# proroklab/DVM-SLAM

Measured on AMD Instinct MI355X. Metric: frames/sec ORB extract+match 640x480x8lvl, higher is better.
Workload: dtype u8; 1 GPU; single agent tracking front end: 640x480 8-level ORB extract (1000 features) + frame-to-frame windowed Hamming match, one agent per GPU; frames_per_launch_group=256, resident_stream_frames=1024, nfeatures=1000, nlevels=8, ini_th_fast=20, min_th_fast=7, match=SearchByProjection(Cur,Last) window th=15, parallelism=agents1, pipeline_lanes=2, stream_texture=rich

## Files before the change

dvm_slam_amd/capi.py:

```python
from __future__ import annotations

import ctypes as C
import os

import numpy as np

_HERE = os.path.dirname(os.path.abspath(__file__))
LIB_PATH = os.environ.get("DVM_HIP_LIB") or os.path.join(_HERE, "lib", "libdvmslam_hip.so")

DVM_OK = 0
ERRORS = {-1: "DVM_ERR_INVALID", -2: "DVM_ERR_EMPTY", -3: "DVM_ERR_CAPACITY", -4: "DVM_ERR_HIP",
          -5: "DVM_ERR_NO_DEVICE", -6: "DVM_ERR_STATE"}

KP_DTYPE = np.dtype([("x", "<f4"), ("y", "<f4"), ("size", "<f4"), ("angle", "<f4"), ("response", "<f4"),
                     ("octave", "<i4"), ("class_id", "<i4")])
MATCH_DTYPE = np.dtype([("best_idx", "<i4"), ("best_dist", "<i4"), ("second_dist", "<i4"),
                        ("best_level", "<i2"), ("second_level", "<i2")])


class DvmError(RuntimeError):
    def __init__(self, code, msg):
        super().__init__(f"{ERRORS.get(code, code)}: {msg}")
        self.code = code

# ... 242 lines not shown
        kps = np.zeros(cap, KP_DTYPE)
        desc = np.zeros((cap, 32), np.uint8)
        n, mono = C.c_int(0), C.c_int(0)
        rc = self.L.dvm_orb_download(self.h, frame, _p(kps), _p(desc), cap, C.byref(n), C.byref(mono))
        if rc == -3 and n.value > cap:
            return self.download(frame, cap=n.value)
        check(rc)
        return n.value, kps[:n.value].copy(), desc[:n.value].copy(), mono.value

    def result_device(self, frame=0):
        k, d, n = C.c_void_p(), C.c_void_p(), C.c_void_p()
        cap = C.c_int(0)
        check(self.L.dvm_orb_result_device(self.h, frame, C.byref(k), C.byref(d), C.byref(n), C.byref(cap)))
        return k.value, d.value, n.value, cap.value

    def copy_result(self, frame, d_kps, d_desc, d_n):
        check(self.L.dvm_orb_copy_result(self.h, frame, C.c_void_p(d_kps), C.c_void_p(d_desc), C.c_void_p(d_n)))

    def scale_factors_device(self):
        return self.L.dvm_orb_scale_factors_device(self.h)

    def pyramid(self, frame, level):
        ptr = C.c_void_p()
        r, c, s = C.c_int(0), C.c_int(0), C.c_int(0)
        check(self.L.dvm_orb_pyramid(self.h, frame, level, C.byref(ptr), C.byref(r), C.byref(c), C.byref(s)))
        return ptr.value, r.value, c.value, s.value

    def debug_level(self, frame, level, bordered=False):
        _, r, c, _ = self.pyramid(frame, level)
        out = np.zeros((r + 38, c + 38) if bordered else (r, c), np.uint8)
        check(self.L.dvm_orb_debug_level(self.h, frame, level, int(bordered), _p(out)))
        return out

    def debug_blurred(self, frame, level):
        _, r, c, _ = self.pyramid(frame, level)
        out = np.zeros((r, c), np.uint8)
        check(self.L.dvm_orb_debug_blurred(self.h, frame, level, _p(out)))
        return out

    def debug_candidates(self, frame, level, cap=300000):
        xs, ys, sc = (np.zeros(cap, np.int32) for _ in range(3))
        n = C.c_int(0)
        check(self.L.dvm_orb_debug_candidates(self.h, frame, level, _p(xs), _p(ys), _p(sc), cap, C.byref(n)))
        return xs[:n.value].copy(), ys[:n.value].copy(), sc[:n.value].copy()

    def debug_level_keypoints(self, frame, level, cap=20000):
        k = np.zeros(cap, KP_DTYPE)
        n = C.c_int(0)
        check(self.L.dvm_orb_debug_level_keypoints(self.h, frame, level, _p(k), cap, C.byref(n)))
        return k[:n.value].copy()

    def profiling(self, on=True):
        check(self.L.dvm_orb_profiling(self.h, int(on)))

    def profile_reset(self):
        check(self.L.dvm_orb_profile_reset(self.h))

    def profile_get(self, name):
        ms, cnt = C.c_double(0), C.c_int64(0)
        rc = self.L.dvm_orb_profile_get(self.h, name.encode(), C.byref(ms), C.byref(cnt))
        return (ms.value, cnt.value) if rc == 0 else (0.0, 0)

    def stream(self):
        return self.L.dvm_orb_stream(self.h)


# ... 1993 lines not shown
```

dvm_slam_amd/csrc/capi.cpp:

```cpp
#include <algorithm>
#include <cstring>
#include <new>
#include <string>
#include <type_traits>
#include <mutex>
#include <unordered_map>
#include <vector>

#include "../../include/dvmslam_hip.h"
#include "camera_model.h"
#include "chain.h"
#include "match_kernels.h"
#include "orb_pipeline.h"

namespace dvm {
const char* last_error_cstr();
}
using namespace dvm;

struct dvm_orb {
  OrbPipeline* p;
  float* d_scale = nullptr;
  uint64_t id = 0, serial = 0;
  int last_n = 0;
// ... 142 lines not shown
}
const float* dvm_orb_scale_factors_device(dvm_orb* h) { return h ? h->d_scale : nullptr; }
int dvm_orb_download(dvm_orb* h, int frame, dvm_keypoint* kps, uint8_t* desc, int cap, int* n, int* mono_index) {
  if (!h) return DVM_ERR_INVALID;
  return h->p->download(frame, kps, desc, cap, n, mono_index);
}
int dvm_orb_download_batch(dvm_orb* h, int count, dvm_keypoint* const* kps, uint8_t* const* desc, const int* caps, int* n, int* mono_index) {
  if (!h || !caps) return DVM_ERR_INVALID;
  return h->p->download_batch(count, kps, desc, caps, n, mono_index);
}
int dvm_orb_pyramid(dvm_orb* h, int frame, int level, const uint8_t** d_ptr, int* rows, int* cols, int* stride) {
  if (!h || !h->p->configured) return DVM_ERR_STATE;
  OrbPipeline& P = *h->p;
  if (level < 0 || level >= P.PD.nlevels || frame < 0 || frame >= P.max_batch) return DVM_ERR_INVALID;
  const LevelDesc& L = P.PD.lv[level];
  if (d_ptr) *d_ptr = P.d_pyr + (size_t)frame * P.PD.pyr_frame_bytes + L.pyr_off + (size_t)kEdge * L.stride + kEdge;
  if (rows) *rows = L.h;
  if (cols) *cols = L.w;
  if (stride) *stride = L.stride;
  return DVM_OK;
}

int dvm_orb_debug_level(dvm_orb* h, int frame, int level, int bordered, uint8_t* out) {
  if (!h || !h->p->configured || !out) return DVM_ERR_STATE;
  OrbPipeline& P = *h->p;
  if (level < 0 || level >= P.PD.nlevels || frame < 0 || frame >= P.last_batch) return DVM_ERR_INVALID;
  int rc = P.sync();
  if (rc != DVM_OK) return rc;
  const LevelDesc& L = P.PD.lv[level];
  const uint8_t* base = P.d_pyr + (size_t)frame * P.PD.pyr_frame_bytes + L.pyr_off;
  if (bordered)
    return hip_check(hipMemcpy2D(out, L.w + 2 * kEdge, base, L.stride, L.w + 2 * kEdge, L.h + 2 * kEdge, hipMemcpyDeviceToHost), "memcpy2d");
  return hip_check(hipMemcpy2D(out, L.w, base + (size_t)kEdge * L.stride + kEdge, L.stride, L.w, L.h, hipMemcpyDeviceToHost), "memcpy2d");
}
int dvm_orb_debug_blurred(dvm_orb* h, int frame, int level, uint8_t* out) {
  if (!h || !h->p->configured || !out) return DVM_ERR_STATE;
  OrbPipeline& P = *h->p;
  if (level < 0 || level >= P.PD.nlevels || frame < 0 || frame >= P.last_batch) return DVM_ERR_INVALID;
  int rc = P.refresh_blur();
  if (rc == DVM_OK) rc = P.sync();
  if (rc != DVM_OK) return rc;
  const LevelDesc& L = P.PD.lv[level];
  return hip_check(hipMemcpy2D(out, L.w, P.d_blur + (size_t)frame * P.PD.blur_frame_bytes + L.blur_off, L.blur_stride, L.w, L.h,
                               hipMemcpyDeviceToHost), "memcpy2d");
}
int dvm_orb_debug_candidates(dvm_orb* h, int frame, int level, int32_t* xs, int32_t* ys, int32_t* scores, int cap, int* n) {
  if (!h || !h->p->configured) return DVM_ERR_STATE;
  OrbPipeline& P = *h->p;
  if (level < 0 || level >= P.PD.nlevels || frame < 0 || frame >= P.last_batch) return DVM_ERR_INVALID;
  int rc = P.sync();
  if (rc != DVM_OK) return rc;
  const LevelDesc& LD = P.PD.lv[level];
  std::vector<int32_t> cc(std::max(LD.cell_count, 1));
  if (LD.cell_count > 0) {
    rc = hip_check(hipMemcpy(cc.data(), P.d_cell_count + (size_t)frame * P.PD.ncells + LD.cell_first, (size_t)LD.cell_count * 4, hipMemcpyDeviceToHost), "memcpy");
    if (rc != DVM_OK) return rc;
  }
  int cnt = 0;
  for (int c = 0; c < LD.cell_count; c++) cnt += cc[c];
  if (n) *n = cnt;
  if (cnt > cap) return DVM_ERR_CAPACITY;
  std::vector<uint32_t> tmp(cnt > 0 ? cnt : 1);
  for (int c = 0, o = 0; c < LD.cell_count; c++) {
    if (cc[c] > 0) {
      rc = hip_check(hipMemcpy(tmp.data() + o, P.d_cand + (size_t)frame * P.PD.cand_frame_slots + P.cells[LD.cell_first + c].cand_base,
                               (size_t)cc[c] * 4, hipMemcpyDeviceToHost), "memcpy");
// ... 986 lines not shown
```

dvm_slam_amd/csrc/orb_kernels.h:

```cpp
#pragma once
#include <hip/hip_runtime.h>
#include <stdint.h>

#include "orb_device.h"

namespace dvm {

struct dvm_keypoint_pod {
  float x, y, size, angle, response;
  int32_t octave, class_id;
};

struct HostMirror {
  dvm_keypoint_pod* kps = nullptr;
  uint8_t* desc = nullptr;
  int32_t* n = nullptr;
  int32_t* mono = nullptr;
};

void upload_constants(const int8_t* disc_u, const int8_t* disc_v, const int* gauss7);
void launch_pyr_level0(hipStream_t s, const uint8_t* d_src, int rows, int cols, int sstride, int64_t frame_stride,
                       uint8_t* d_pyr, const PipelineDesc& PD, int batch);
void launch_pyr_resize(hipStream_t s, uint8_t* d_pyr, const PipelineDesc& PD, int level, const int32_t* d_tabs, int batch);
void launch_pyr_borders(hipStream_t s, uint8_t* d_pyr, const PipelineDesc& PD, int batch);
void launch_fast(hipStream_t s, const uint8_t* d_pyr, const CellDesc* d_cells, const PipelineDesc& PD, uint32_t* d_cand,
                 int32_t* d_cell_count, int batch, int max_rw, int max_rh, int cell_first, int cell_num, const CellDesc* h_cells);
int octree_root_nodes(const LevelDesc& L);
bool raise_dynamic_lds(const void* fn, int bytes);
bool octree_fits_device(const PipelineDesc& PD);
bool octree_prepare_device(const PipelineDesc& PD);
void launch_octree(hipStream_t s, const uint32_t* d_cand, const int32_t* d_cell_count, const CellDesc* d_cells, uint32_t* d_dense,
                   int32_t* d_lvl_count, const PipelineDesc& PD, int32_t* d_nid, uint32_t* d_sel, int32_t* d_nsel, int32_t* d_err,
                   int batch, int level_first, int level_num, bool latency = false);
bool octree_blur_fits(const PipelineDesc& PD);
void launch_octree_blur(hipStream_t s, const uint32_t* d_cand, const int32_t* d_cell_count, const CellDesc* d_cells, uint32_t* d_dense,
                        int32_t* d_lvl_count, const PipelineDesc& PD, int32_t* d_nid, uint32_t* d_sel, int32_t* d_nsel, int32_t* d_err, int batch,
                        const uint8_t* d_pyr, uint8_t* d_blur, const TileDesc* d_tiles, const int* gauss7);
void launch_assemble(hipStream_t s, const uint32_t* d_sel, const int32_t* d_nsel, const PipelineDesc& PD, int lap0,
                     int lap1, dvm_keypoint_pod* d_kps, KpAux* d_aux, int32_t* d_n, int32_t* d_mono, int batch,
                     HostMirror hm = HostMirror());
void launch_blur(hipStream_t s, const uint8_t* d_pyr, uint8_t* d_blur, const TileDesc* d_tiles, const PipelineDesc& PD,
                 const int32_t* d_lvl_start, int batch);
void launch_orient_desc(hipStream_t s, const uint8_t* d_pyr, const uint8_t* d_blur, const PipelineDesc& PD,
                        const KpAux* d_aux, const int32_t* d_n, dvm_keypoint_pod* d_kps, uint8_t* d_desc, int batch,
                        HostMirror hm = HostMirror());
void launch_orient_desc_blur(hipStream_t s, const uint8_t* d_pyr, const PipelineDesc& PD, const KpAux* d_aux, const int32_t* d_n,
                             dvm_keypoint_pod* d_kps, uint8_t* d_desc, int batch, HostMirror hm = HostMirror());
void launch_copy_result(hipStream_t s, const dvm_keypoint_pod* kps_src, dvm_keypoint_pod* kps_dst, const uint8_t* desc_src, uint8_t* desc_dst, int cap,
                        const int32_t* n_src, int32_t* n_dst);

}
```

dvm_slam_amd/csrc/orb_kernels.hip:

```cpp
#include <hip/hip_runtime.h>

#include <map>
#include <mutex>
#include <utility>

#include <algorithm>
#include <cstdlib>

#include "orb_device.h"
#include "orb_kernels.h"
#include "blur_tile.h"

#pragma clang fp contract(off)

namespace dvm {

__constant__ int c_pattern[1024] = {
#include "orb_pattern_31.inc"
};
__constant__ int8_t c_circle[16][2] = {{0, 3},  {1, 3},   {2, 2},   {3, 1},   {3, 0},  {3, -1}, {2, -2}, {1, -3},
                                       {0, -3}, {-1, -3}, {-2, -2}, {-3, -1}, {-3, 0}, {-3, 1}, {-2, 2}, {-1, 3}};
__device__ uint2 c_disc_w[256];
__device__ uint2 c_disc_w43[512];
__constant__ int c_gauss7[7];
// ... 164 lines not shown
  if (X4 >= bw) return;
  uint8_t* Dl = pyr + (int64_t)f * pyr_frame_bytes + L.pyr_off;
#pragma unroll
  for (int rr = 0; rr < TH / 4; rr++) {
    const int dy = y0 + ty + 4 * rr;
    if (dy >= L.h) break;
    const int sy = sy_[rr];
    const int r0 = min(max(sy, 0), P.h - 1) - sya, r1 = min(max(sy + 1, 0), P.h - 1) - sya;
    const uint32_t bb = bb_[rr];
    const uint32_t b0 = bb & 0xFFFFu, b1 = bb >> 16;
    const uint8_t* S0 = rz_smem + r0 * lds_pitch;
    const uint8_t* S1 = rz_smem + r1 * lds_pitch;
    uint32_t v = 0;
#pragma unroll
    for (int k = 0; k < 4; k++) {
      const uint32_t s00 = S0[sx[k]], s01 = S0[sx[k] + 1], s10 = S1[sx[k]], s11 = S1[sx[k] + 1];
      const uint32_t h0 = udot2(s00 | (s01 << 16), al[k], 0u);
      const uint32_t h1 = udot2(s10 | (s11 << 16), al[k], 0u);
      const uint32_t r = ((__umul24(b0, h0 >> 4) >> 16) + (__umul24(b1, h1 >> 4) >> 16) + 2u) >> 2;
      v |= r << (8 * k);
    }
    *reinterpret_cast<uint32_t*>(Dl + (int64_t)(kEdge + dy) * L.stride + X4) = v;
    int top, bot;
    mirror_rows(dy, L.h, top, bot);
    if (top >= 0) *reinterpret_cast<uint32_t*>(Dl + (int64_t)top * L.stride + X4) = v;
    if (bot >= 0) *reinterpret_cast<uint32_t*>(Dl + (int64_t)bot * L.stride + X4) = v;
  }
}

template <int TH>
__global__ void __launch_bounds__(256) k_pyr_resize(uint8_t* __restrict__ pyr, int pyr_frame_bytes, LevelDesc P,
                                                    LevelDesc L, const int32_t* __restrict__ tabs, int lds_pitch) {
  pyr_resize_tile<TH>(pyr, pyr_frame_bytes, P, L, tabs, lds_pitch, blockIdx.z, blockIdx.x, blockIdx.y);
}

__global__ void __launch_bounds__(256) k_pyr_borders(uint8_t* __restrict__ pyr, PipelineDesc PD, int strip_blocks) {
  const int f = blockIdx.z, tid = threadIdx.x;
  if ((int)blockIdx.y < strip_blocks) {
    const int sr = blockIdx.y * 4 + (tid >> 6);
    if (sr >= 2 * kEdge * PD.nlevels) return;
    const LevelDesc& L = PD.lv[sr / (2 * kEdge)];
    const int r = sr % (2 * kEdge);
    const int row = r < kEdge ? r : L.h + r;
    const int X = 32 + (blockIdx.x * 64 + (tid & 63)) * 16;
    if (X + 16 > L.w + kEdge) return;
    uint8_t* base = pyr + (int64_t)f * PD.pyr_frame_bytes + L.pyr_off;
    const uint8_t* S = base + (int64_t)(kEdge + reflect101(row - kEdge, L.h)) * L.stride;
    *reinterpret_cast<uint4*>(base + (int64_t)row * L.stride + X) = *reinterpret_cast<const uint4*>(S + X);
    return;
  }
  if (blockIdx.x != 0) return;
  int g = ((int)blockIdx.y - strip_blocks) * 128 + (tid >> 1), lvl = 0;
  while (lvl < PD.nlevels && g >= PD.lv[lvl].h + 2 * kEdge) { g -= PD.lv[lvl].h + 2 * kEdge; lvl++; }
  if (lvl >= PD.nlevels) return;
  const LevelDesc& L = PD.lv[lvl];
  const int w = L.w;
  const bool strip = g < kEdge || g >= L.h + kEdge;
  uint8_t* base = pyr + (int64_t)f * PD.pyr_frame_bytes + L.pyr_off;
  uint8_t* D = base + (int64_t)g * L.stride;
  const uint8_t* S = base + (int64_t)(kEdge + reflect101(g - kEdge, L.h)) * L.stride;
  uint32_t* D32 = reinterpret_cast<uint32_t*>(D);
  const uint32_t* S32 = reinterpret_cast<const uint32_t*>(S);
  if (w < 40) {
    if (tid & 1) return;
    for (int X = 0; X < w + 2 * kEdge; X++)
      if (strip || X < kEdge || X >= w + kEdge) D[X] = S[kEdge + reflect101(X - kEdge, w)];
// ... 1019 lines not shown
  uint2 w[256];
  for (int i = 0; i < 256; i++) w[i] = make_uint2(0u, 0u);
  for (int p = 0; p < kDiscPixels; p++) {
    const int u = disc_u[p], v = disc_v[p];
    const int item = (v + kHalfPatch) * 8 + ((u + kHalfPatch) >> 2), k = (u + kHalfPatch) & 3;
    w[item].x |= (uint32_t)(u + 16) << (8 * k);
    w[item].y |= 1u << (8 * k);
  }
  hipMemcpyToSymbol(HIP_SYMBOL(c_disc_w), w, sizeof(w));
  uint2 w43[512];
  for (int i = 0; i < 512; i++) w43[i] = make_uint2(0u, 0u);
  for (int p = 0; p < kDiscPixels; p++) {
    const int u = disc_u[p], v = disc_v[p];
    const int item = (v + kPbR) * kPbDw + ((u + kPbR) >> 2), k = (u + kPbR) & 3;
    w43[item].x |= (uint32_t)(u + 16) << (8 * k);
    w43[item].y |= 1u << (8 * k);
  }
  hipMemcpyToSymbol(HIP_SYMBOL(c_disc_w43), w43, sizeof(w43));
  hipMemcpyToSymbol(HIP_SYMBOL(c_gauss7), gauss7, 7 * sizeof(int));
}

void launch_pyr_level0(hipStream_t s, const uint8_t* d_src, int rows, int cols, int sstride, int64_t frame_stride,
                       uint8_t* d_pyr, const PipelineDesc& PD, int batch) {
  const LevelDesc& L = PD.lv[0];
  dim3 grid(cdiv(cdiv(L.w + 2 * kEdge, 16), 64), cdiv(L.h, 16), batch);
  hipLaunchKernelGGL(k_pyr_level0, grid, dim3(256), 0, s, d_src, rows, cols, sstride, frame_stride, d_pyr,
                     PD.pyr_frame_bytes, L);
}
void launch_pyr_resize(hipStream_t s, uint8_t* d_pyr, const PipelineDesc& PD, int level, const int32_t* d_tabs, int batch) {
  const LevelDesc& L = PD.lv[level];
  const LevelDesc& P = PD.lv[level - 1];
  const double sxs = (double)P.w / L.w, sys = (double)P.h / L.h;
  const int pitch = (((int)(kRzTW * sxs) + 16) + 3) & ~3;
  if (batch <= 8) {
    const int nrows = (int)(16 * sys) + 4;
    dim3 grid(cdiv(L.w + 2 * kEdge, kRzTW), cdiv(L.h, 16), batch);
    hipLaunchKernelGGL(k_pyr_resize<16>, grid, dim3(256), (size_t)pitch * nrows, s, d_pyr, PD.pyr_frame_bytes, P, L, d_tabs, pitch);
    return;
  }
  const int nrows = (int)(kRzTH * sys) + 4;
  dim3 grid(cdiv(L.w + 2 * kEdge, kRzTW), cdiv(L.h, kRzTH), batch);
  hipLaunchKernelGGL(k_pyr_resize<kRzTH>, grid, dim3(256), (size_t)pitch * nrows, s, d_pyr, PD.pyr_frame_bytes, P, L, d_tabs, pitch);
}
void launch_pyr_borders(hipStream_t s, uint8_t* d_pyr, const PipelineDesc& PD, int batch) {
  int rows = 0, maxw = 0;
  for (int l = 0; l < PD.nlevels; l++) { rows += PD.lv[l].h + 2 * kEdge; maxw = std::max(maxw, PD.lv[l].w + 2 * kEdge); }
  const int strip_blocks = cdiv(2 * kEdge * PD.nlevels, 4);
  dim3 grid(std::max(1, cdiv(cdiv(maxw, 16), 64)), strip_blocks + cdiv(rows, 128), batch);
  hipLaunchKernelGGL(k_pyr_borders, grid, dim3(256), 0, s, d_pyr, PD, strip_blocks);
}
static void launch_fast_wide(hipStream_t s, const uint8_t* d_pyr, const CellDesc* d_cells, const PipelineDesc& PD, uint32_t* d_cand,
                             int32_t* d_cell_count, int batch, int max_rw, int max_rh, int cell_first, int cell_num) {
  const FastLds lay = fast_lds_layout(max_rw, max_rh);
  const dim3 grid(cell_num * 8 * ((batch + 8 * kFastFramesPerWG - 1) / (8 * kFastFramesPerWG)));
  const bool small = (max_rw - 6) * (max_rh - 6) <= 32 * 128;
  static const int lds_pad = std::getenv("DVM_FAST_LDS_PAD") ? atoi(std::getenv("DVM_FAST_LDS_PAD")) : 0;
#define DVM_FAST_LAUNCH(P, W)                                                                                              \
  do {                                                                                                                     \
    if (lay.total() > 48 * 1024)                                                                                           \
      raise_dynamic_lds(reinterpret_cast<const void*>(k_fast_cells<P, W>), lay.total());                                   \
    hipLaunchKernelGGL((k_fast_cells<P, W>), grid, dim3(64 * W), lay.total() + lds_pad, s, d_pyr, PD.pyr_frame_bytes, d_cells, PD,   \
                       d_cand, d_cell_count, max_rw, max_rh, batch, cell_first, cell_num);                                 \
  } while (0)
  if (lay.tile_pitch == 64) { if (small) DVM_FAST_LAUNCH(64, 2); else DVM_FAST_LAUNCH(64, 4); }
  else DVM_FAST_LAUNCH(0, 4);
#undef DVM_FAST_LAUNCH
}
void launch_fast(hipStream_t s, const uint8_t* d_pyr, const CellDesc* d_cells, const PipelineDesc& PD, uint32_t* d_cand,
                 int32_t* d_cell_count, int batch, int max_rw, int max_rh, int cell_first, int cell_num, const CellDesc* h_cells) {
  if (cell_num <= 0) return;
  static const int lds1_max = std::getenv("DVM_FAST1_LDS") ? atoi(std::getenv("DVM_FAST1_LDS")) : 5120;
  static const int lds1_max64 = std::getenv("DVM_FAST1_LDS64") ? atoi(std::getenv("DVM_FAST1_LDS64")) : 0;
  if (!h_cells || lds1_max <= 0) { launch_fast_wide(s, d_pyr, d_cells, PD, d_cand, d_cell_count, batch, max_rw, max_rh, cell_first, cell_num); return; }
  const int end = cell_first + cell_num;
  int run_first = cell_first, run_kind = -1, run_rw = 0, run_rh = 0;
// ... 77 lines not shown
```

dvm_slam_amd/csrc/orb_pipeline.cpp:

```cpp
#include "orb_pipeline.h"
#include "chain.h"
#include "host_stage.h"

#include <algorithm>
#include <cmath>
#include <cstdlib>
#include <cstring>
#include <mutex>
#include <thread>

namespace dvm {

static thread_local std::string g_err;
void set_error(const std::string& msg) { g_err = msg; }
const char* last_error_cstr() { return g_err.c_str(); }
int hip_check(hipError_t e, const char* what) {
  if (e == hipSuccess) return DVM_OK;
  set_error(std::string(what) + ": " + hipGetErrorString(e));
  return DVM_ERR_HIP;
}

hipEvent_t Profiler::get_event() {
  if (!pool_.empty()) {
    hipEvent_t e = pool_.back();
// ... 228 lines not shown
}

int OrbPipeline::init() {
  { const int rc = need_device(device); if (rc != DVM_OK) return rc; }
  DVM_HIP(hipStreamCreateWithFlags(&stream, hipStreamNonBlocking));
  lane_main[0] = stream;
  if (const char* e = getenv("DVM_BLUR_EARLY")) blur_early = (e[0] == '1');
  if (const char* e = getenv("DVM_GROUPS")) sscanf(e, "%d,%d", &group_split[0], &group_split[1]);
  if (const char* e = getenv("DVM_CHUNKS")) chunks = std::min(std::max(atoi(e), 1), (int)kMaxChunks);
  {
    int least = 0, greatest = 0;
    DVM_HIP(hipDeviceGetStreamPriorityRange(&least, &greatest));
    side_priority = least;
    if (chunks > 1 || group_split[0] < kMaxLevels) {
      DVM_HIP(hipStreamCreateWithPriority(&lane_side[1], hipStreamNonBlocking, least));
      DVM_HIP(hipStreamCreateWithFlags(&lane_main[1], hipStreamNonBlocking));
    }
    (void)greatest;
  }
  DVM_HIP(hipEventCreateWithFlags(&ev_start, hipEventDisableTiming));
  DVM_HIP(hipEventCreateWithFlags(&ev_done, hipEventDisableTiming));
  for (int g = 0; g < 4; g++) DVM_HIP(hipEventCreateWithFlags(&ev_group[g], hipEventDisableTiming));
  for (int c = 0; c < kMaxChunks; c++) {
    DVM_HIP(hipEventCreateWithFlags(&ev_compact[c], hipEventDisableTiming));
    DVM_HIP(hipEventCreateWithFlags(&ev_fork[c], hipEventDisableTiming));
    DVM_HIP(hipEventCreateWithFlags(&ev_join[c], hipEventDisableTiming));
  }
  if (const char* e = getenv("DVM_LATENCY_PATH")) latency_path = (e[0] != '0');
  if (const char* e = getenv("DVM_OCT_BLUR")) oct_blur = (e[0] != '0');
  if (const char* e = getenv("DVM_LAT_SPLIT")) lat_split = (e[0] != '0');
  if (const char* e = getenv("DVM_ZERO_COPY_IN")) zero_copy_in = (e[0] != '0');
  if (const char* e = getenv("DVM_SERIAL")) overlap_blur = (e[0] != '1');
  if (const char* e = getenv("DVM_PATCH_BLUR")) patch_blur = (e[0] != '0');
#ifdef DVM_DEBUG
  if (const char* e = getenv("DVM_HOST_OCTREE")) host_octree_forced = (e[0] == '1');
#endif
  host_octree = host_octree_forced;
  int8_t du[kDiscPixels], dv[kDiscPixels];
  int n = 0;
  for (int v = -kHalfPatch; v <= kHalfPatch; v++) {
    const int d = umax[std::abs(v)];
    for (int u = -d; u <= d; u++) { du[n] = (int8_t)u; dv[n] = (int8_t)v; n++; }
  }
  if (n != kDiscPixels) { set_error("disc size mismatch"); return DVM_ERR_STATE; }
  int g7[7];
  {
    double k[7], s = 0;
    for (int i = 0; i < 7; i++) { double x = i - 3.0; k[i] = std::exp(-0.5 / 4.0 * x * x); s += k[i]; }
    double err = 0; long long acc = 0;
    for (int i = 0; i < 3; i++) {
      double adj = k[i] * (1.0 / s) * 256.0 + err;
      long long v = (long long)std::nearbyint(adj);
      err = adj - (double)v;
      g7[i] = g7[6 - i] = (int)v;
      acc += v;
    }
    g7[3] = (int)(256 - 2 * acc);
  }
  for (int i = 0; i < 7; i++) gauss7[i] = g7[i];
  upload_constants(du, dv, g7);
  DVM_HIP(hipGetLastError());
  DVM_HIP(hipDeviceSynchronize());
  return DVM_OK;
}

void OrbPipeline::free_all() {
// ... 41 lines not shown
  std::memset(&PD, 0, sizeof(PD));
  PD.nlevels = L; PD.rows = rows; PD.cols = cols;
  PD.ini_th = std::min(std::max(params.ini_th_fast, 0), 255);
  PD.min_th = std::min(std::max(params.min_th_fast, 0), 255);
  cells.clear(); tiles.clear();
  std::vector<int32_t> tabs;
  int pyr_off = 0, blur_off = 0, cand_off = 0, sel_off = 0;
  for (int l = 0; l < L; l++) {
    LevelDesc& D = PD.lv[l];
    D.w = cv_round_f((float)cols * inv_scale[l]);
    D.h = cv_round_f((float)rows * inv_scale[l]);
    if (D.w < 1 || D.h < 1) { set_error("pyramid level collapses to zero size"); return DVM_ERR_INVALID; }
    D.stride = align_up(D.w + 2 * kEdge, 64);
    D.pyr_off = pyr_off;
    pyr_off += align_up(D.stride * (D.h + 2 * kEdge), 256);
    D.blur_stride = align_up(D.w, 64);
    D.blur_off = blur_off;
    blur_off += align_up(D.blur_stride * D.h, 256);
    D.scale = scale[l];
    D.patch_size = (int)(31 * scale[l]);
    D.quota = nfeat[l];
    D.sel_off = sel_off;
    D.sel_cap = std::max(std::max(nfeat[l], 1), 4 * std::max(octree_root_nodes(D), 0)) + 4;
    sel_off += D.sel_cap;
    if (l > 0) {
      std::vector<int32_t> xo, xa, yo, yb;
      resize_axis_tables(PD.lv[l - 1].w, D.w, true, xo, xa);
      resize_axis_tables(PD.lv[l - 1].h, D.h, false, yo, yb);
      D.tab_off = (int)tabs.size();
      tabs.insert(tabs.end(), xo.begin(), xo.end());
      tabs.insert(tabs.end(), xa.begin(), xa.end());
      tabs.insert(tabs.end(), yo.begin(), yo.end());
      tabs.insert(tabs.end(), yb.begin(), yb.end());
    }
    D.cell_first = (int)cells.size();
    cand_off = align_up(cand_off, 32);
    D.cand_off = cand_off;
    const int minBX = kEdge - 3, minBY = minBX, maxBX = D.w - kEdge + 3, maxBY = D.h - kEdge + 3;
    const float width = (float)(maxBX - minBX), height = (float)(maxBY - minBY);
    const float W = 35;
    const int nCols = (int)(width / W), nRows = (int)(height / W);
    if (nCols > 0 && nRows > 0) {
      const int wCell = (int)std::ceil(width / nCols), hCell = (int)std::ceil(height / nRows);
      for (int i = 0; i < nRows; i++) {
        const float iniY = (float)(minBY + i * hCell);
        float maxY = iniY + hCell + 6;
        if (iniY >= maxBY - 3) continue;
        if (maxY > maxBY) maxY = (float)maxBY;
        for (int j = 0; j < nCols; j++) {
          const float iniX = (float)(minBX + j * wCell);
          float maxX = iniX + wCell + 6;
          if (iniX >= maxBX - 6) continue;
          if (maxX > maxBX) maxX = (float)maxBX;
          CellDesc c{};
          c.level = (int16_t)l;
          c.x0 = (int16_t)iniX; c.y0 = (int16_t)iniY;
          c.rw = (int16_t)((int)maxX - (int)iniX); c.rh = (int16_t)((int)maxY - (int)iniY);
          if (c.rw > kMaxCellDim || c.rh > kMaxCellDim) { set_error("FAST cell larger than supported"); return DVM_ERR_INVALID; }
          const int ew = std::max(c.rw - 6, 0), eh = std::max(c.rh - 6, 0);
          c.cand_cap = ((ew + 1) / 2) * ((eh + 1) / 2);
          c.cand_base = cand_off;
          cand_off += c.cand_cap;
          cells.push_back(c);
        }
      }
    }
// ... 162 lines not shown
  last_mirrored = small;
  if (small) {
    hm = mirror_dev;
  }
  const bool fused = patch_blur && !small;
  blur_stale = fused;
  const bool blur_first = blur_early && !small;
  const bool split0 = small && lat_split && overlap_blur && !host_octree && !tiny_levels && L > 1 && chunks == 1 && group_split[0] >= L;
  if (split0 && !lat_aux) DVM_HIP(hipStreamCreateWithFlags(&lat_aux, hipStreamNonBlocking));

  int nck = host_octree ? 1 : std::min(chunks, std::max(1, batch / 32));
  auto run_half = [&](hipStream_t st, hipStream_t side, int ck, int f0, int nb) -> int {
    uint8_t* pyr_f0 = d_pyr + (size_t)f0 * PD.pyr_frame_bytes;
    uint32_t* cand_f0 = d_cand + (size_t)f0 * PD.cand_frame_slots;
    int32_t* cnt_f0 = d_cell_count + (size_t)f0 * PD.ncells;
    prof.begin(st, "pyramid");
    launch_pyr_level0(st, d_imgs + (int64_t)f0 * frame_stride, rows, cols, stride, frame_stride, pyr_f0, PD, nb);
    uint32_t* dense_f0 = d_dense + (size_t)f0 * PD.cand_frame_slots;
    int32_t* lcnt_f0 = d_lvl_count + (size_t)f0 * kMaxLevels;
    int32_t* nid_f0 = d_nid + (size_t)f0 * PD.cand_frame_slots;
    uint32_t* sel_f0 = d_sel + (size_t)f0 * PD.sel_frame_slots;
    int32_t* nsel_f0 = d_nsel + (size_t)f0 * L;
    if (split0) {
      DVM_HIP(hipEventRecord(ev_group[0], st));
      DVM_HIP(hipStreamWaitEvent(lat_aux, ev_group[0], 0));
      launch_fast(lat_aux, pyr_f0, d_cells, PD, cand_f0, cnt_f0, nb, max_cell_rw, max_cell_rh, PD.lv[0].cell_first, PD.lv[0].cell_count, cells.data());
      launch_octree(lat_aux, cand_f0, cnt_f0, d_cells, dense_f0, lcnt_f0, PD, nid_f0, sel_f0, nsel_f0, d_err, nb, 0, 1, true);
      DVM_HIP(hipEventRecord(ev_group[3], lat_aux));
    }
    if (d_imgs == d_stage && ev_stage_free && f0 + nb >= batch) {
      DVM_HIP(hipEventRecord(ev_stage_free, st));
      stage_free_valid = true;
    }
    for (int l = 1; l < L; l++) launch_pyr_resize(st, pyr_f0, PD, l, d_tabs, nb);
    if (tiny_levels) launch_pyr_borders(st, pyr_f0, PD, nb);
    prof.end(st);
    const bool blur_forked = overlap_blur && !host_octree && side != nullptr && !small && !fused;
    if (blur_forked && blur_first) {
      DVM_HIP(hipEventRecord(ev_fork[ck], st));
      DVM_HIP(hipStreamWaitEvent(side, ev_fork[ck], 0));
      prof.begin(side, "blur");
      launch_blur(side, pyr_f0, (d_blur + (size_t)f0 * PD.blur_frame_bytes), d_tiles, PD, nullptr, nb);
      prof.end(side);
      DVM_HIP(hipEventRecord(ev_join[ck], side));
    }
    hipStream_t aux = lane_main[st == lane_main[0] ? 1 : 0];
    const bool grouped = overlap_blur && !host_octree && chunks == 1 && aux != nullptr && group_split[0] < L;
    const int g_a = std::min(std::max(group_split[0], 0), L), g_b = std::min(std::max(group_split[1], g_a), L);
    const int gl[4] = {split0 ? 1 : 0, grouped ? g_a : L, grouped ? g_b : L, L};
    int oct_main_first = split0 ? 1 : 0;
    bool blur_done = false;
    prof.begin(st, "fast");
    for (int gi = 0; gi < 3; gi++) {
      const int la = gl[gi], lb = gl[gi + 1];
      if (la >= lb) continue;
      const int c_first = PD.lv[la].cell_first, c_end = PD.lv[lb - 1].cell_first + PD.lv[lb - 1].cell_count;
      launch_fast(st, pyr_f0, d_cells, PD, cand_f0, cnt_f0, nb, max_cell_rw, max_cell_rh, c_first, c_end - c_first, cells.data());
      if (grouped && lb < L) {
        DVM_HIP(hipEventRecord(ev_group[gi], st));
        DVM_HIP(hipStreamWaitEvent(aux, ev_group[gi], 0));
        launch_octree(aux, cand_f0, cnt_f0, d_cells, dense_f0, lcnt_f0, PD, nid_f0, sel_f0, nsel_f0, d_err, nb, la, lb - la, small);
        oct_main_first = lb;
      }
    }
    prof.end(st);
    if (nck > 1) DVM_HIP(hipEventRecord(ev_compact[ck], st));
    auto fork_blur = [&]() -> int {
// ... 203 lines not shown
```

dvm_slam_amd/csrc/orb_pipeline.h:

```cpp
#pragma once
#include <hip/hip_runtime.h>

#include <map>
#include <string>
#include <vector>

#include "../../include/dvmslam_hip.h"
#include "orb_device.h"
#include "orb_kernels.h"

namespace dvm {

void set_error(const std::string& msg);
const char* last_error_cstr();
int hip_check(hipError_t e, const char* what);
#define DVM_HIP(call)                                  \
  do {                                                 \
    int _rc = ::dvm::hip_check((call), #call);         \
    if (_rc != DVM_OK) return _rc;                     \
  } while (0)

class Profiler {
 public:
  bool enabled = false;
// ... 19 lines not shown

class OrbPipeline {
 public:
  OrbPipeline(const dvm_orb_params& p, int device, int max_batch);
  ~OrbPipeline();
  int init();
  int extract_device(const uint8_t* d_imgs, int batch, int rows, int cols, int stride, int64_t frame_stride, int lap0,
                     int lap1);
  int extract_host(const uint8_t* imgs, int batch, int rows, int cols, int stride, int64_t frame_stride, int lap0,
                   int lap1);
  int ensure_stage(size_t need);
  hipStream_t copy_stream = nullptr;
  hipEvent_t ev_copied = nullptr, ev_stage_free = nullptr;
  bool copy_pending = false, stage_free_valid = false;
  int staging(int batch, int rows, int cols, uint8_t** host_ptr);
  int extract_staged(int batch, int rows, int cols, int lap0, int lap1);
  int extract_staged_sync_owner(int batch, int rows, int cols, int lap0, int lap1);
  int sync();
  int download(int frame, dvm_keypoint* kps, uint8_t* desc, int cap, int* n, int* mono);

  dvm_orb_params params;
  int device, max_batch;
  hipStream_t stream = nullptr;
  static constexpr int kMaxChunks = 8;
  hipStream_t lane_main[2] = {nullptr, nullptr}, lane_side[2] = {nullptr, nullptr};
  int group_split[2] = {kMaxLevels, kMaxLevels};
  hipEvent_t ev_group[4] = {};
  hipEvent_t ev_start = nullptr, ev_compact[kMaxChunks] = {}, ev_fork[kMaxChunks] = {}, ev_join[kMaxChunks] = {}, ev_done = nullptr;
  int chunks = 1;
  bool blur_early = true;
  bool overlap_blur = true;
  int side_priority = 0;
  bool patch_blur = true;
  bool blur_stale = false;
  int refresh_blur();
  Profiler prof;
  std::vector<float> scale, inv_scale, sigma2, inv_sigma2;
  std::vector<int> nfeat;
  int umax[16];

  PipelineDesc PD{};
  std::vector<CellDesc> cells;
  std::vector<TileDesc> tiles;
  int last_batch = 0;
  int max_cell_rw = 8, max_cell_rh = 8;
  bool tiny_levels = false;
  bool configured = false;

  uint8_t* d_pyr = nullptr;
  uint8_t* d_blur = nullptr;
  int32_t* d_tabs = nullptr;
  CellDesc* d_cells = nullptr;
  TileDesc* d_tiles = nullptr;
  uint32_t* d_cand = nullptr;
  uint32_t* d_dense = nullptr;
  int32_t* d_cell_count = nullptr;
  int32_t* d_lvl_count = nullptr;
  uint32_t* d_sel = nullptr;
  int32_t* d_nsel = nullptr;
  dvm_keypoint_pod* d_kps = nullptr;
  uint8_t* d_desc = nullptr;
  KpAux* d_aux = nullptr;
  int32_t* d_n = nullptr;
  int32_t* d_mono = nullptr;
  int32_t* d_nid = nullptr;
  int32_t* d_err = nullptr;
// ... 35 lines not shown
```

include/dvmslam_hip.h:

```cpp
#ifndef DVMSLAM_HIP_H
#define DVMSLAM_HIP_H
#include <stdint.h>
#ifdef __cplusplus
extern "C" {
#endif

typedef enum {
  DVM_OK = 0,
  DVM_ERR_INVALID = -1,
  DVM_ERR_EMPTY = -2,
  DVM_ERR_CAPACITY = -3,
  DVM_ERR_HIP = -4,
  DVM_ERR_NO_DEVICE = -5,
  DVM_ERR_STATE = -6
} dvm_status;

const char* dvm_last_error(void);
const char* dvm_version(void);
int dvm_device_count(void);
int dvm_set_device(int device);

typedef struct {
  float x, y, size, angle, response;
  int32_t octave, class_id;
// ... 19 lines not shown
int dvm_orb_pool_create(const dvm_orb_params* p, int device, int max_batch, int window_us, dvm_orb_pool** out);
void dvm_orb_pool_destroy(dvm_orb_pool* pool);
int dvm_orb_pool_extract(dvm_orb_pool* pool, const uint8_t* img, int rows, int cols, int stride, int lap0, int lap1, dvm_keypoint* kps,
                         uint8_t* desc, int cap, int* n, int* mono_index, int* batch_size);

int dvm_orb_extract_batch_device(dvm_orb* h, const uint8_t* d_imgs, int batch, int rows, int cols, int stride,
                                 int64_t frame_stride, int lap0, int lap1);
int dvm_orb_extract_batch_host(dvm_orb* h, const uint8_t* imgs, int batch, int rows, int cols, int stride,
                               int64_t frame_stride, int lap0, int lap1);
int dvm_orb_staging(dvm_orb* h, int batch, int rows, int cols, uint8_t** host_ptr);
int dvm_orb_extract_staged(dvm_orb* h, int batch, int rows, int cols, int lap0, int lap1);
int dvm_orb_sync(dvm_orb* h);
int dvm_orb_result_device(dvm_orb* h, int frame, const dvm_keypoint** d_kps, const uint8_t** d_desc,
                          const int32_t** d_n, int* capacity);
typedef struct {
  const dvm_keypoint* d_kps;
  const uint8_t* d_desc;
  int32_t n, device;
  uint64_t handle_id, serial;
} dvm_device_frame;
int dvm_orb_last_result(dvm_orb* h, dvm_device_frame* out);
int dvm_device_frame_valid(const dvm_device_frame* ref);
int dvm_orb_copy_result(dvm_orb* h, int frame, dvm_keypoint* d_kps_dst, uint8_t* d_desc_dst, int32_t* d_n_dst);
const float* dvm_orb_scale_factors_device(dvm_orb* h);
int dvm_orb_download(dvm_orb* h, int frame, dvm_keypoint* kps, uint8_t* desc, int cap, int* n, int* mono_index);
int dvm_orb_download_batch(dvm_orb* h, int count, dvm_keypoint* const* kps, uint8_t* const* desc, const int* caps, int* n, int* mono_index);
int dvm_orb_pyramid(dvm_orb* h, int frame, int level, const uint8_t** d_ptr, int* rows, int* cols, int* stride);

int dvm_orb_debug_level(dvm_orb* h, int frame, int level, int bordered, uint8_t* out );
int dvm_orb_debug_blurred(dvm_orb* h, int frame, int level, uint8_t* out);
int dvm_orb_debug_candidates(dvm_orb* h, int frame, int level, int32_t* xs, int32_t* ys, int32_t* scores,
                             int cap, int* n);
int dvm_orb_debug_level_keypoints(dvm_orb* h, int frame, int level, dvm_keypoint* kps, int cap, int* n);

int dvm_orb_profiling(dvm_orb* h, int enable);
int dvm_orb_profile_get(dvm_orb* h, const char* name, double* total_ms, int64_t* launches);
int dvm_orb_profile_reset(dvm_orb* h);
void* dvm_orb_stream(dvm_orb* h);

int dvm_hamming_matrix(const uint8_t* A, int nA, const uint8_t* B, int nB, uint16_t* D, int on_device, void* stream);

typedef struct dvm_frame dvm_frame;
int dvm_frame_create(int device, int capacity, int slots, dvm_frame** out);
void dvm_frame_destroy(dvm_frame* f);
int dvm_frame_build(dvm_frame* f, int slot, const dvm_keypoint* kps, const uint8_t* desc, int n, const int32_t* d_n,
                    float minX, float maxX, float minY, float maxY, int on_device, void* stream);
int dvm_frame_build_batch(dvm_frame* f, int first_slot, int count, const dvm_keypoint* d_kps, int64_t kps_stride,
                          const uint8_t* d_desc, int64_t desc_stride, const int32_t* d_n, float minX, float maxX,
                          float minY, float maxY, void* stream);
int dvm_frame_overflows(dvm_frame* f, int32_t* count);

typedef struct {
  int32_t best_idx;
  int32_t best_dist;
  int32_t second_dist;
  int16_t best_level, second_level;
} dvm_match;

int dvm_match_window(const dvm_frame* train, int slot, const uint8_t* skip, const uint8_t* qdesc, const float* qx,
                     const float* qy, const float* qr, const int32_t* qmin, const int32_t* qmax, int nq,
                     const int32_t* d_nq, dvm_match* out, int on_device, void* stream);
int dvm_match_window_top2(const dvm_frame* train, int slot, const uint8_t* skip, const uint8_t* qdesc, const float* qx,
                          const float* qy, const float* qr, const int32_t* qmin, const int32_t* qmax, int nq,
                          const int32_t* d_nq, dvm_match* out, int32_t* second_idx, int on_device, void* stream);
int dvm_match_window_ranked(const dvm_frame* train, int slot, const uint8_t* skip, const uint8_t* qdesc, const float* qx, const float* qy,
                            const float* qr, const int32_t* qmin, const int32_t* qmax, int nq, uint32_t* ranked, int on_device, void* stream);
// ... 440 lines not shown
```

Before: 300,800 frames/s.

## Add direct register-window pyramid resize kernel for large batches

Adds a new pyramid downscale kernel that works without LDS. Each wave keeps a sliding window of source rows in registers, gathers the needed bytes with perm instructions and does the bilinear interpolation with packed dot products. It writes the output rows and their mirrored border rows directly. A host-side check validates the lookup tables and picks a strip height per level. The new kernel is used when the batch exceeds the latency batch size, and the old tiled LDS kernel remains the fallback. The aim is to cut LDS staging and syncs in the resize stage, at the risk of extra redundant source reads and lower occupancy from the register window.

```diff
diff --git a/dvm_slam_amd/capi.py b/dvm_slam_amd/capi.py
--- a/dvm_slam_amd/capi.py
+++ b/dvm_slam_amd/capi.py
@@ -298,6 +298,13 @@
         check(self.L.dvm_orb_debug_level(self.h, frame, level, int(bordered), _p(out)))
         return out
 
+    def debug_pyr_path(self, level) -> int:
+        out = C.c_int(0)
+        f = self.L.dvm_orb_debug_pyr_path
+        f.restype = C.c_int32; f.argtypes = None
+        check(f(self.h, C.c_int32(level), C.byref(out)))
+        return out.value
+
     def debug_blurred(self, frame, level):
         _, r, c, _ = self.pyramid(frame, level)
         out = np.zeros((r, c), np.uint8)
diff --git a/dvm_slam_amd/csrc/capi.cpp b/dvm_slam_amd/csrc/capi.cpp
--- a/dvm_slam_amd/csrc/capi.cpp
+++ b/dvm_slam_amd/csrc/capi.cpp
@@ -198,6 +198,13 @@
   if (bordered)
     return hip_check(hipMemcpy2D(out, L.w + 2 * kEdge, base, L.stride, L.w + 2 * kEdge, L.h + 2 * kEdge, hipMemcpyDeviceToHost), "memcpy2d");
   return hip_check(hipMemcpy2D(out, L.w, base + (size_t)kEdge * L.stride + kEdge, L.stride, L.w, L.h, hipMemcpyDeviceToHost), "memcpy2d");
+}
+int dvm_orb_debug_pyr_path(dvm_orb* h, int level, int* out) {
+  if (!h || !h->p->configured || !out) return DVM_ERR_STATE;
+  OrbPipeline& P = *h->p;
+  if (level < 0 || level >= P.PD.nlevels) return DVM_ERR_INVALID;
+  *out = P.pyr_path[level];
+  return DVM_OK;
 }
 int dvm_orb_debug_blurred(dvm_orb* h, int frame, int level, uint8_t* out) {
   if (!h || !h->p->configured || !out) return DVM_ERR_STATE;
diff --git a/dvm_slam_amd/csrc/orb_kernels.h b/dvm_slam_amd/csrc/orb_kernels.h
--- a/dvm_slam_amd/csrc/orb_kernels.h
+++ b/dvm_slam_amd/csrc/orb_kernels.h
@@ -22,6 +22,9 @@
 void launch_pyr_level0(hipStream_t s, const uint8_t* d_src, int rows, int cols, int sstride, int64_t frame_stride,
                        uint8_t* d_pyr, const PipelineDesc& PD, int batch);
 void launch_pyr_resize(hipStream_t s, uint8_t* d_pyr, const PipelineDesc& PD, int level, const int32_t* d_tabs, int batch);
+constexpr int kRzLatencyBatch = 8;
+int pyr_direct_strip_rows(const LevelDesc& P, const LevelDesc& L, const int32_t* xofs, const int32_t* yofs);
+void launch_pyr_resize_direct(hipStream_t s, uint8_t* d_pyr, const PipelineDesc& PD, int level, const int32_t* d_tabs, int batch, int strip_rows);
 void launch_pyr_borders(hipStream_t s, uint8_t* d_pyr, const PipelineDesc& PD, int batch);
 void launch_fast(hipStream_t s, const uint8_t* d_pyr, const CellDesc* d_cells, const PipelineDesc& PD, uint32_t* d_cand,
                  int32_t* d_cell_count, int batch, int max_rw, int max_rh, int cell_first, int cell_num, const CellDesc* h_cells);
diff --git a/dvm_slam_amd/csrc/orb_kernels.hip b/dvm_slam_amd/csrc/orb_kernels.hip
--- a/dvm_slam_amd/csrc/orb_kernels.hip
+++ b/dvm_slam_amd/csrc/orb_kernels.hip
@@ -220,6 +220,95 @@
 __global__ void __launch_bounds__(256) k_pyr_resize(uint8_t* __restrict__ pyr, int pyr_frame_bytes, LevelDesc P,
                                                     LevelDesc L, const int32_t* __restrict__ tabs, int lds_pitch) {
   pyr_resize_tile<TH>(pyr, pyr_frame_bytes, P, L, tabs, lds_pitch, blockIdx.z, blockIdx.x, blockIdx.y);
+}
+
+#ifndef DVM_PYR_NS
+#define DVM_PYR_NS 24
+#endif
+#ifndef DVM_PYR_WAVES
+#define DVM_PYR_WAVES 4
+#endif
+constexpr int kRdNS = DVM_PYR_NS;
+constexpr int kRdWaves = DVM_PYR_WAVES;
+__device__ __forceinline__ uint32_t mul_hi_u24(uint32_t a, uint32_t b) {
+  return (uint32_t)(((uint64_t)(a & 0xFFFFFFu) * (uint64_t)(b & 0xFFFFFFu)) >> 32);
+}
+template <int NS>
+__global__ void __launch_bounds__(64 * kRdWaves) k_pyr_resize_direct(uint8_t* __restrict__ pyr, int pyr_frame_bytes, LevelDesc P, LevelDesc L,
+                                                           const int32_t* __restrict__ tabs, int R) {
+  const int f = blockIdx.z, tx = threadIdx.x & 63;
+  const int ty = __builtin_amdgcn_readfirstlane(threadIdx.x >> 6);
+  const int w = L.w, bw = L.w + 2 * kEdge;
+  const int y0 = ((int)blockIdx.y * kRdWaves + ty) * R;
+  if (y0 >= L.h) return;
+  const int yl = min(y0 + R - 1, L.h - 1);
+  const int Xt = ((int)blockIdx.x * 64 + tx) * 4;
+  const bool live = Xt < bw;
+  const int X4 = live ? Xt : ((bw - 1) & ~3);
+  const int32_t* xofs = tabs + L.tab_off;
+  const int32_t* xal = xofs + L.w;
+  const int32_t* yofs = xal + L.w;
+  const int32_t* ybe = yofs + L.h;
+  const int dyl = min(y0 + tx, yl);
+  const int yv = yofs[dyl];
+  const uint32_t bv = (uint32_t)ybe[dyl];
+  int sx[4];
+  uint32_t al[4];
+#pragma unroll
+  for (int k = 0; k < 4; k++) {
+    const int x = min(X4 + k, bw - 1) - kEdge;
+    const int xm = x < 0 ? -x : (x >= w ? 2 * (w - 1) - x : x);
+    sx[k] = xofs[xm];
+    al[k] = (uint32_t)xal[xm];
+  }
+  const int base = min(min(sx[0], sx[1]), min(sx[2], sx[3]));
+  uint32_t sel[4];
+#pragma unroll
+  for (int k = 0; k < 4; k++) sel[k] = 0x0c000c00u | (uint32_t)(sx[k] - base) | ((uint32_t)(sx[k] + 1 - base) << 16);
+  const int sya = __builtin_amdgcn_readlane(yv, 0);
+  const int syb = __builtin_amdgcn_readlane(yv, (yl - y0) & 63) + 1;
+  const uint8_t* Sf = pyr + (int64_t)f * pyr_frame_bytes + P.pyr_off;
+  const uint32_t scol = (uint32_t)(kEdge + base);
+  uint2 win[NS];
+#pragma unroll
+  for (int j = 0; j < NS; j++) {
+    const uint8_t* Sr = Sf + (uint32_t)((kEdge + min(sya + j, syb)) * P.stride);
+    __builtin_memcpy(&win[j], Sr + scol, 8);
+  }
+  uint8_t* Dl = pyr + (int64_t)f * pyr_frame_bytes + L.pyr_off;
+  int d = y0;
+  int syd = __builtin_amdgcn_readlane(yv, 0);
+  uint32_t bbd = __builtin_amdgcn_readlane(bv, 0);
+  int r1 = syd + 1;
+  uint32_t prev[4] = {0u, 0u, 0u, 0u}, cur[4];
+#pragma unroll
+  for (int j = 0; j < NS; j++) {
+    if (sya + j > syb) break;
+#pragma unroll
+    for (int k = 0; k < 4; k++) cur[k] = udot2(__builtin_amdgcn_perm(win[j].y, win[j].x, sel[k]), al[k], 0u) & 0xFFFFF0u;
+    if (d <= yl && r1 == sya + j) {
+      const uint32_t b0 = (bbd & 0xFFFFu) << 12, b1 = (bbd >> 16) << 12;
+      uint32_t v = 0;
+#pragma unroll
+      for (int k = 0; k < 4; k++) {
+        const uint32_t r = (mul_hi_u24(b0, prev[k]) + mul_hi_u24(b1, cur[k]) + 2u) >> 2;
+        v |= r << (8 * k);
+      }
+      if (live) {
+        *reinterpret_cast<uint32_t*>(Dl + (int64_t)(kEdge + d) * L.stride + X4) = v;
+        int top, bot;
+        mirror_rows(d, L.h, top, bot);
+        if (top >= 0) *reinterpret_cast<uint32_t*>(Dl + (int64_t)top * L.stride + X4) = v;
+        if (bot >= 0) *reinterpret_cast<uint32_t*>(Dl + (int64_t)bot * L.stride + X4) = v;
+      }
+      d++;
+      syd = __builtin_amdgcn_readlane(yv, (d - y0) & 63);
+      bbd = __builtin_amdgcn_readlane(bv, (d - y0) & 63);
+      r1 = syd + 1;
+    }
+#pragma unroll
+    for (int k = 0; k < 4; k++) prev[k] = cur[k];
+  }
 }
 
 __global__ void __launch_bounds__(256) k_pyr_borders(uint8_t* __restrict__ pyr, PipelineDesc PD, int strip_blocks) {
@@ -1305,7 +1394,7 @@
   const LevelDesc& P = PD.lv[level - 1];
   const double sxs = (double)P.w / L.w, sys = (double)P.h / L.h;
   const int pitch = (((int)(kRzTW * sxs) + 16) + 3) & ~3;
-  if (batch <= 8) {
+  if (batch <= kRzLatencyBatch) {
     const int nrows = (int)(16 * sys) + 4;
     dim3 grid(cdiv(L.w + 2 * kEdge, kRzTW), cdiv(L.h, 16), batch);
     hipLaunchKernelGGL(k_pyr_resize<16>, grid, dim3(256), (size_t)pitch * nrows, s, d_pyr, PD.pyr_frame_bytes, P, L, d_tabs, pitch);
@@ -1314,6 +1403,37 @@
   const int nrows = (int)(kRzTH * sys) + 4;
   dim3 grid(cdiv(L.w + 2 * kEdge, kRzTW), cdiv(L.h, kRzTH), batch);
   hipLaunchKernelGGL(k_pyr_resize<kRzTH>, grid, dim3(256), (size_t)pitch * nrows, s, d_pyr, PD.pyr_frame_bytes, P, L, d_tabs, pitch);
+}
+int pyr_direct_strip_rows(const LevelDesc& P, const LevelDesc& L, const int32_t* xofs, const int32_t* yofs) {
+  if (L.w < 40 || L.h < 20 || P.w < 40 || P.h < 20) return 0;
+  const int w = L.w, bw = L.w + 2 * kEdge;
+  for (int X4 = 0; X4 < bw; X4 += 4) {
+    int lo = INT32_MAX, hi = INT32_MIN;
+    for (int k = 0; k < 4; k++) {
+      const int x = std::min(X4 + k, bw - 1) - kEdge;
+      const int xm = x < 0 ? -x : (x >= w ? 2 * (w - 1) - x : x);
+      if (xm < 0 || xm >= w) return 0;
+      lo = std::min(lo, xofs[xm]);
+      hi = std::max(hi, xofs[xm] + 1);
+    }
+    if (lo < 0 || hi - lo + 1 > 8 || kEdge + lo + 8 > P.stride) return 0;
+  }
+  for (int y = 0; y < L.h; y++) {
+    if (yofs[y] < 0 || yofs[y] + 1 > P.h - 1) return 0;
+    if (y > 0 && yofs[y] <= yofs[y - 1]) return 0;
+  }
+  for (int R = std::min(kRdNS, 63); R >= 1; R--) {
+    bool ok = true;
+    for (int y0 = 0; y0 < L.h && ok; y0 += R) ok = yofs[std::min(y0 + R - 1, L.h - 1)] + 1 - yofs[y0] + 1 <= kRdNS;
+    if (ok) return R;
+  }
+  return 0;
+}
+void launch_pyr_resize_direct(hipStream_t s, uint8_t* d_pyr, const PipelineDesc& PD, int level, const int32_t* d_tabs, int batch, int strip_rows) {
+  const LevelDesc& L = PD.lv[level];
+  const LevelDesc& P = PD.lv[level - 1];
+  dim3 grid(cdiv(cdiv(L.w + 2 * kEdge, 4), 64), cdiv(cdiv(L.h, strip_rows), kRdWaves), batch);
+  hipLaunchKernelGGL(k_pyr_resize_direct<kRdNS>, grid, dim3(64 * kRdWaves), 0, s, d_pyr, PD.pyr_frame_bytes, P, L, d_tabs, strip_rows);
 }
 void launch_pyr_borders(hipStream_t s, uint8_t* d_pyr, const PipelineDesc& PD, int batch) {
   int rows = 0, maxw = 0;
diff --git a/dvm_slam_amd/csrc/orb_pipeline.cpp b/dvm_slam_amd/csrc/orb_pipeline.cpp
--- a/dvm_slam_amd/csrc/orb_pipeline.cpp
+++ b/dvm_slam_amd/csrc/orb_pipeline.cpp
@@ -284,6 +284,7 @@
   if (const char* e = getenv("DVM_ZERO_COPY_IN")) zero_copy_in = (e[0] != '0');
   if (const char* e = getenv("DVM_SERIAL")) overlap_blur = (e[0] != '1');
   if (const char* e = getenv("DVM_PATCH_BLUR")) patch_blur = (e[0] != '0');
+  if (const char* e = getenv("DVM_PYR_DIRECT")) pyr_direct = (e[0] != '0');
 #ifdef DVM_DEBUG
   if (const char* e = getenv("DVM_HOST_OCTREE")) host_octree_forced = (e[0] == '1');
 #endif
@@ -391,6 +392,7 @@
       tabs.insert(tabs.end(), xa.begin(), xa.end());
       tabs.insert(tabs.end(), yo.begin(), yo.end());
       tabs.insert(tabs.end(), yb.begin(), yb.end());
+      pyr_strip[l] = pyr_direct ? pyr_direct_strip_rows(PD.lv[l - 1], D, xo.data(), yo.data()) : 0;
     }
     D.cell_first = (int)cells.size();
     cand_off = align_up(cand_off, 32);
@@ -619,7 +621,11 @@
       DVM_HIP(hipEventRecord(ev_stage_free, st));
       stage_free_valid = true;
     }
-    for (int l = 1; l < L; l++) launch_pyr_resize(st, pyr_f0, PD, l, d_tabs, nb);
+    for (int l = 1; l < L; l++) {
+      pyr_path[l] = nb > kRzLatencyBatch && pyr_strip[l] > 0;
+      if (pyr_path[l]) launch_pyr_resize_direct(st, pyr_f0, PD, l, d_tabs, nb, pyr_strip[l]);
+      else launch_pyr_resize(st, pyr_f0, PD, l, d_tabs, nb);
+    }
     if (tiny_levels) launch_pyr_borders(st, pyr_f0, PD, nb);
     prof.end(st);
     const bool blur_forked = overlap_blur && !host_octree && side != nullptr && !small && !fused;
diff --git a/dvm_slam_amd/csrc/orb_pipeline.h b/dvm_slam_amd/csrc/orb_pipeline.h
--- a/dvm_slam_amd/csrc/orb_pipeline.h
+++ b/dvm_slam_amd/csrc/orb_pipeline.h
@@ -75,6 +75,9 @@
   bool overlap_blur = true;
   int side_priority = 0;
   bool patch_blur = true;
+  bool pyr_direct = true;
+  int pyr_strip[kMaxLevels] = {};
+  uint8_t pyr_path[kMaxLevels] = {};
   bool blur_stale = false;
   int refresh_blur();
   Profiler prof;
diff --git a/include/dvmslam_hip.h b/include/dvmslam_hip.h
--- a/include/dvmslam_hip.h
+++ b/include/dvmslam_hip.h
@@ -75,6 +75,7 @@
 int dvm_orb_debug_candidates(dvm_orb* h, int frame, int level, int32_t* xs, int32_t* ys, int32_t* scores,
                              int cap, int* n);
 int dvm_orb_debug_level_keypoints(dvm_orb* h, int frame, int level, dvm_keypoint* kps, int cap, int* n);
+int dvm_orb_debug_pyr_path(dvm_orb* h, int level, int* out);
 
 int dvm_orb_profiling(dvm_orb* h, int enable);
 int dvm_orb_profile_get(dvm_orb* h, const char* name, double* total_ms, int64_t* launches);
```

Measured after the change: 308,500 frames/s, median of 6. +2.6%, better.
